# mit-han-lab/llm-awq

Measured on AMD Instinct MI355X. Metric: W4A16 decode+prefill tok/s, Llama-3-8B; achieved %HBM (GEMV) / %MFMA (GEMM), higher is better.
Workload: dtype bf16; 1 GPU; Llama-3-8B W4A16 g128 bf16 activations on 1xMI355X (decode GEMV + prefill GEMM); layers=32, decode_m=1, prefill_m=2048, graph=True, layout=cdna4, clock_ramp_steps=60, decode_mlp=gate/up + SiLU*mul launch, then down_proj, prefill_mlp=SiLU*mul fused into the gate/up GEMM epilogue, mlp=interleaved, decode_side_buffer=sz_half, parallelism=tp1, full=False

## Files before the change

### llm_awq_amd/csrc/awq_gemv_dma.hip

```cpp
#include <string.h>

#include <type_traits>
#include <utility>

#include "../../include/awq_cdna4.h"
#include "awq_device.hpp"
#include "awq_dma.hpp"
#include "awq_kernels.hpp"

namespace awq {

#ifdef AWQ_ENABLE_PROBES
#define DMA_PROBE(p) ((p) & 0xFF)
#else
#define DMA_PROBE(p) 0
#endif
constexpr int kDmaF32Out = 0x100;
constexpr int kDmaInterleave = 0x200;
template <typename DT, int WAVES, int EPI, int NS>
__device__ __forceinline__ void gemv_dma_reduce(char* smem, char* wbase, int wave_bytes, const f32x4 (&acc)[NS], const uint16_t* __restrict__ bias,
                                                uint16_t* __restrict__ out, int M, int N, int probe_, int nb, int lane, int wv) {
  const int i = lane & 15, g = lane >> 4;
#pragma unroll
  for (int s = 0; s < NS; ++s)
// ... 366 lines not shown
  if (wide8 && !g_dma_want) want = tx > 4 ? 2 : 3;
  if (g_dma_d) d = g_dma_d < tx ? g_dma_d : tx;
  while (d > 1 && dma_smem(waves, d, ns, tx, m) * want > 156 * 1024) --d;
  if (d == 3) d = 2;
  if (d == 5 || d == 6 || (d == 7 && waves == 8)) d = 4;
  if (d == 8 && waves == 16) d = 7;
  c = {waves, tx, d, dma_smem(waves, d, ns, tx, m)};
  return c.smem <= 160 * 1024 && tx >= d;
}
}

int gemv_dma_tune_set(const char* key, int value) {
  if (!strcmp(key, "gemvd_waves")) g_dma_waves = value;
  else if (!strcmp(key, "gemvd_d")) g_dma_d = value;
  else if (!strcmp(key, "gemvd_probe")) g_dma_probe = value;
  else if (!strcmp(key, "gemvd_four")) g_dma_four = value;
  else if (!strcmp(key, "gemvd_want")) g_dma_want = value;
  else if (!strcmp(key, "gemvd_wide8")) g_dma_wide8 = value;
  else if (!strcmp(key, "gemvd_il")) g_dma_il = value;
  else if (!strcmp(key, "decode_skinny_small")) g_dma_skinny_small = value;
  else if (!strcmp(key, "decode_skinny_m1")) g_dma_skinny_m1 = value;
  else if (!strcmp(key, "decode_skinny_from")) g_dma_skinny_from = value;
  else return -1;
  return 0;
}

template <typename DT, int WAVES, int D, int DQ, int EPI>
static void launch_dma_cfg(const void* x, const void* qw, const void* szp, const void* bias, void* out, int m, int n, int k,
                           const DmaCfg& c, hipStream_t st, int f32out) {
  constexpr int NS = EPI == 1 ? 2 : 1;
  const int flags = (g_dma_probe & 0xFF) | (f32out ? kDmaF32Out : 0) | ((g_dma_il == 1 || (g_dma_il == 2 && c.d < c.tx && c.waves == 8)) ? kDmaInterleave : 0);
  constexpr int TXC = EPI == 1 ? 0 : ((WAVES == 8 && (D == 2 || D == 4)) ? 4 : ((WAVES == 16 && D == 1) ? 7 : 0));
  if constexpr (TXC != 0) {
    if (m == 1 && c.tx == TXC && k == WAVES * TXC * kGroup) {
      auto kern1 = gemv_dma_kernel_m1<DT, WAVES, D, DQ, EPI, TXC>;
      static LdsOptIn optin1;
      if (c.smem > 64 * 1024) optin1.ensure(reinterpret_cast<const void*>(kern1));
      hipLaunchKernelGGL(kern1, dim3(n / 16 / NS), dim3(64 * WAVES), c.smem, st, (const uint16_t*)x, (const u32*)qw, (const u32*)szp,
                         (const uint16_t*)bias, (uint16_t*)out, m, n, k, c.tx, flags);
      return;
    }
  }
  auto kern = gemv_dma_kernel<DT, WAVES, D, DQ, EPI>;
  static LdsOptIn optin;
  if (c.smem > 64 * 1024) optin.ensure(reinterpret_cast<const void*>(kern));
  hipLaunchKernelGGL(kern, dim3(n / 16 / NS), dim3(64 * WAVES), c.smem, st, (const uint16_t*)x, (const u32*)qw, (const u32*)szp,
                     (const uint16_t*)bias, (uint16_t*)out, m, n, k, c.tx, flags);
}

template <typename DT, int EPI, int DQ>
static int launch_dma_dt(const void* x, const void* qw, const void* szp, const void* bias, void* out, int m, int n, int k,
                         hipStream_t st, int f32out) {
  DmaCfg c;
  if (!pick_dma(m, n, k, EPI == 1 ? 2 : 1, c)) return -1;
#define AWQ_DCASE(W_, D_)                                                           \
  if (c.waves == W_ && c.d == D_) {                                                 \
    launch_dma_cfg<DT, W_, D_, DQ, EPI>(x, qw, szp, bias, out, m, n, k, c, st, f32out); \
    return 0;                                                                       \
  }
  AWQ_DCASE(8, 1) AWQ_DCASE(8, 2) AWQ_DCASE(8, 4) AWQ_DCASE(8, 8)
  AWQ_DCASE(16, 1) AWQ_DCASE(16, 2) AWQ_DCASE(16, 4) AWQ_DCASE(16, 7)
  AWQ_DCASE(4, 1) AWQ_DCASE(4, 2) AWQ_DCASE(4, 4) AWQ_DCASE(4, 7) AWQ_DCASE(4, 8)
#undef AWQ_DCASE
  return -1;
}

int gemv_dma_plan(int m, int n, int k, int epi, int* kernel) {
  if (m < 1 || m > 8 || k < 128 || (k % 128) != 0 || epi < 0 || epi > 2 || n < (epi == 1 ? 32 : 16) || (n % (epi == 1 ? 32 : 16)) != 0) return 0;
  if (skinny_takes(m, n, k, epi)) {
    if (kernel) *kernel = 1;
    return 1;
  }
  if (kernel) *kernel = 0;
  DmaCfg c;
  int mc = m;
  while (mc > 1 && !pick_dma(mc, n, k, epi == 1 ? 2 : 1, c)) --mc;
  if (!pick_dma(mc, n, k, epi == 1 ? 2 : 1, c)) return 0;
  return (m + mc - 1) / mc;
}

int launch_gemv_dma(const void* x, const void* qw, const void* szp, const void* bias, void* out, int m, int n, int k, int epi,
                    int dtype, int szfmt, hipStream_t st, int f32out) {
  if (m < 1 || m > 8 || (k % 128) != 0 || (n % (epi == 1 ? 32 : 16)) != 0 || (f32out && (epi != 0 || bias != nullptr))) return -1;
  if (skinny_takes(m, n, k, epi) && launch_skinny_decode(x, qw, szp, bias, out, m, n, k, epi, dtype, szfmt, st, f32out) == 0) return 0;
  DmaCfg probe_cfg;
  int mc = m;
  while (mc > 1 && !pick_dma(mc, n, k, epi == 1 ? 2 : 1, probe_cfg)) --mc;
  if (mc < m) {
    if (!pick_dma(mc, n, k, epi == 1 ? 2 : 1, probe_cfg)) return -1;
    const size_t ncols = epi ? (size_t)n / 2 : (size_t)n;
    for (int r = 0; r < m; r += mc) {
      const int rows = m - r < mc ? m - r : mc;
      const int rc = launch_gemv_dma((const char*)x + (size_t)r * k * 2, qw, szp, bias, (char*)out + (size_t)r * ncols * (f32out ? 4 : 2), rows, n, k,
                                     epi, dtype, szfmt, st, f32out);
      if (rc != 0) return rc;
    }
    return 0;
  }
#define AWQ_DDT(DT_, DQ_)                                                                   \
  if (epi == 0) return launch_dma_dt<DT_, 0, DQ_>(x, qw, szp, bias, out, m, n, k, st, f32out); \
  if (epi == 1) return launch_dma_dt<DT_, 1, DQ_>(x, qw, szp, bias, out, m, n, k, st, 0);      \
  return launch_dma_dt<DT_, 2, DQ_>(x, qw, szp, bias, out, m, n, k, st, 0);
  if (szfmt == 1) {
    if (dtype == 0) {
      AWQ_DDT(F16, 1)
    }
    AWQ_DDT(BF16, 1)
  }
  if (dtype == 0) {
    AWQ_DDT(F16, 0)
  }
  AWQ_DDT(BF16, 0)
#undef AWQ_DDT
}

}
```

### llm_awq_amd/csrc/awq_kernels.hpp

```cpp
#pragma once
#include <hip/hip_runtime.h>
#include <stddef.h>
#include <stdint.h>

#include <atomic>

namespace awq {
struct LdsOptIn {
  std::atomic<uint64_t> done[4] = {};
  void ensure(const void* kern, int bytes = 160 * 1024) {
    int dev = 0;
    (void)hipGetDevice(&dev);
    const uint64_t bit = 1ull << (dev & 63);
    std::atomic<uint64_t>& w = done[(dev >> 6) & 3];
    if (w.load(std::memory_order_acquire) & bit) return;
    (void)hipFuncSetAttribute(kern, hipFuncAttributeMaxDynamicSharedMemorySize, bytes);
    w.fetch_or(bit, std::memory_order_release);
  }
};
inline int device_cu_count() {
  static std::atomic<int> cached[64] = {};
  int dev = 0;
  if (hipGetDevice(&dev) != hipSuccess) return 256;
  std::atomic<int>& c = cached[dev & 63];
  int v = c.load(std::memory_order_relaxed);
  if (v == 0) {
    if (hipDeviceGetAttribute(&v, hipDeviceAttributeMultiprocessorCount, dev) != hipSuccess || v <= 0) v = 256;
    c.store(v, std::memory_order_relaxed);
  }
  return v;
}
int launch_gemv(const void* x, const void* qw, const void* s, const void* z, const void* szp, void* out, int m, int n,
                int k, int dtype, int layout, hipStream_t st);
int launch_gemv_cdna4(const void* x, const void* qw, const void* szp, const void* bias, void* out, int m, int n, int k,
                      int epi, int bits, int dtype, hipStream_t st);
int launch_gemv_cdna4_norm(const void* x, const void* gamma, float eps, const void* qw, const void* szp, const void* bias, void* out,
                           int m, int n, int k, int epi, int dtype, hipStream_t st);
bool gemv_v2fast_enabled();
int launch_gemv_v2fast(const void* x, const void* qw, const void* s, const void* z, const void* bias, void* out, int m, int n, int k,
                       int gpad, int dtype, hipStream_t st);
int launch_skinny_v2(const void* x, const void* qw, const void* s, const void* z, const void* bias, void* out, int m, int n, int k,
                     int gpad, int dtype, hipStream_t st);
int launch_pack_w3(const void* q_u8, void* qw3, int n, int k, hipStream_t st);
int launch_unpack_w3(const void* qw3, void* out_u8, int n, int k, hipStream_t st);
int launch_dequant_w3(const void* qw3, const void* s, const void* z, void* out, int n, int k, int dtype, hipStream_t st);
int launch_expand_w3_to_cdna4(const void* qw3, void* qw4, int n, int k, hipStream_t st);
int gemv_cdna4_tune_set(const char* key, int value);
int launch_gemv_dma(const void* x, const void* qw, const void* szp, const void* bias, void* out, int m, int n, int k, int epi,
                    int dtype, int szfmt, hipStream_t st, int f32out = 0);
int gemv_dma_tune_set(const char* key, int value);
int launch_moe_gemv_cdna4(const void* x, const void* qw, const void* szp, const void* offsets, void* out, int total_rows,
                          int experts, int n, int k, int dtype, hipStream_t st);
int launch_moe_skinny_tail_cdna4(const void* x, const void* qw, const void* szp, const void* offsets, void* out, int experts, int n, int k,
                                 int dtype, hipStream_t st, int epi, int tail);
void moe_v6_set_tail(int v);
int launch_moe_skinny_cdna4(const void* x, const void* qw, const void* szp, const void* offsets, void* out, int total_rows,
                            int experts, int n, int k, int dtype, hipStream_t st);
int launch_pack_sz_cdna4(const void* s, const void* z, void* szp, int n, int k, hipStream_t st);
int launch_pack_szh_cdna4(const void* s, const void* z, void* szh, int* inexact, int n, int k, int dtype, hipStream_t st);
int launch_gemm(const void* x, const void* qw, const void* s, const void* z, const void* szp, void* out, int m, int n,
                int k, int dtype, int layout, void* ws, size_t ws_bytes, hipStream_t st);
int launch_repack_v2_cdna4(const void* src, void* dst, int n, int k, int to_cdna4, hipStream_t st);
int launch_unpack_cdna4(const void* qw, void* out_u8, int n, int k, hipStream_t st);
int launch_dequant_cdna4(const void* qw, const void* s, const void* z, void* out, int n, int k, int dtype, hipStream_t st);
size_t gemm_workspace_bytes(int m, int n, int k);
int launch_gemm_cdna4_v3(const void* x, const void* qw, const void* szp, const void* bias, void* out, int m, int n, int k,
                         int tile_n, int dtype, void* ws, size_t ws_bytes, hipStream_t st, int bits = 4, int epi = 0, const void* szh = nullptr);
int gemm_variant_get();
int launch_skinny_cdna4(const void* x, const void* qw, const void* szp, const void* bias, void* out, int m, int n, int k,
                        int dtype, hipStream_t st, int f32out = 0, void* ws = nullptr, size_t ws_bytes = 0);
int launch_skinny_w3(const void* x, const void* qw, const void* szp, const void* bias, void* out, int m, int n, int k, int epi, int dtype, hipStream_t st,
                     int f32out = 0);
int launch_skinny_gate_up(const void* x, const void* qw, const void* szp, void* out, int m, int n2, int k, int dtype, hipStream_t st);
int skinny_splitk_parts(int m, int n, int k);
size_t skinny_splitk_workspace_bytes(int m, int n, int k);
int skinny_tune_set(const char* key, int value);
int launch_midm_cdna4(const void* x, const void* qw, const void* szp, const void* bias, void* out, int m, int n, int k, int epi, int dtype, int szfmt,
                      int bits, int f32out, void* ws, size_t ws_bytes, hipStream_t st);
bool midm_takes(int m, int n, int k);
size_t midm_workspace_bytes(int m, int n, int k);
int midm_parts(int m, int n, int k);
int midm_tune_set(const char* key, int value);
int midm_init();
unsigned* splitk_ticket_words(hipStream_t st, int groups);
int launch_skinny_decode(const void* x, const void* qw, const void* szp, const void* bias, void* out, int m, int n, int k, int epi,
                         int dtype, int szfmt, hipStream_t st, int f32out = 0);
int launch_moe_gemm(const void* x, const void* qw, const void* s, const void* z, const void* offsets, void* out, int total_m,
                    int experts, int n, int k, int gpad, int dtype, int layout, hipStream_t st);
int gemv_tune_set(const char* key, int value);
int gemm_tune_set(const char* key, int value);
int gemm_v3_tune_set(const char* key, int value);
void launch_gemm_cdna4_v4n(const void* x, const void* qw, const void* szp, const void* bias, void* out, int m, int n, int k,
                           int n_begin, int n_end, int dtype, void* ws, size_t ws_bytes, hipStream_t st, int bits = 4, int epi = 0);
size_t gemm_v4n_workspace_bytes(int m, int n_cols, int k);
extern int g_v4n_ksplit_force;
extern int g_v4n_ksplit_cap;
bool gemm_cdna4_v3_takes(int m, int k);
size_t gemm_cdna4_v3_workspace_bytes(int m, int n, int k);
int gemm_cdna4_v3_plan(int m, int n, int bits, int* mode, int* cols_main);
int gemm_cdna4_v3_narrow_kernel(int m, int n_cols, int k, int bits, int has_workspace, int epi);
int gemv_dma_plan(int m, int n, int k, int epi, int* kernel);
size_t gemm_cdna4_v3_workspace_bytes_w3(int m, int n, int k);
bool moe_v4_enabled();
int launch_moe_gemm_cdna4_v6(const void* x, const void* qw, const void* szp, const void* offsets, void* out, int total, int experts,
                             int n, int k, int dtype, hipStream_t st, int epi = 0, const void* szh = nullptr);
int launch_silu_mul_interleaved(const void* in, void* out, int m, int n2, int dtype, hipStream_t st);
int launch_silu_mul(const void* gate, const void* up, void* out, size_t count, int dtype, hipStream_t st);
bool moe_v6_enabled();
int launch_moe_route(const void* logits, int logits_dtype, int tokens, int experts, int top_k, int renormalize, void* topk_ids, void* topk_w,
                     void* order, void* inv, void* offsets, hipStream_t st);
int launch_moe_gather(const void* x, const void* order, void* xs, int tokens, int top_k, int hidden, hipStream_t st);
int launch_moe_combine(const void* ys, const void* inv, const void* topk_w, void* out, int tokens, int top_k, int hidden, int dtype, hipStream_t st);
int launch_sample_logits(const void* logits, int logits_dtype, int batch, int vocab, const void* u, const void* temperature, const void* top_k,
                         const void* top_p, const void* penalty, void* history, void* hist_len, int max_history, void* seqlens, const void* stop_ids,
                         int num_stop, void* finished, int max_len, int flags, void* tokens, hipStream_t st);
int launch_spec_draft_ngram(const void* history, const void* hist_len, const void* seqlens, const void* max_draft, void* drafts, void* draft_len,
                            int batch, int max_history, int vocab, int kmax, int ngram_min, int ngram_max, int max_len, hipStream_t st);
int launch_spec_pack(const void* last_tokens, void* drafts, void* draft_len, const void* seqlens, void* cu_seqlens_q, void* input_ids, int batch,
                     int kmax, int total_q, hipStream_t st);
int launch_spec_verify(const void* logits, int logits_dtype, int total_q, int vocab, const void* u, const void* cu_seqlens_q, const void* input_ids,
                       int batch, const void* temperature, const void* top_k, const void* top_p, const void* penalty, const void* history,
                       const void* hist_len, int max_history, void* row_tokens, hipStream_t st);
int launch_spec_accept(const void* row_tokens, const void* input_ids, const void* cu_seqlens_q, int batch, int total_q, int kmax, void* history,
                       void* hist_len, int max_history, void* seqlens, const void* stop_ids, int num_stop, void* finished, int max_len, int flags,
                       void* out_tokens, void* num_emitted, void* last_tokens, hipStream_t st);
int lm_head_plan(int m, int v, int k, int out[4]);
int launch_lm_head(const void* x, long ldx, const void* gamma, float eps, const void* weight, const void* bias, const int* seqlens, void* out,
                   int out_f32, int m, int v, int k, int dtype, int max_blocks, hipStream_t st);
int launch_embed_tokens(const int* tokens, const void* table, void* out, int n, int v, int k, hipStream_t st);
int lora_plan(int k, int r, int n_slices, int out[4]);
size_t lora_workspace_bytes(int total_q, int k, int r, int n_slices);
int launch_lora_shrink(const void* x, long ldx, const void* a_pool, const int* adapter_ids, const int* cu_seqlens_q, void* ws, int batch,
                       int max_seqlen_q, int total_q, int slots, int k, int r, int n_slices, int dtype, hipStream_t st);
int launch_lora_expand(const void* ws, const void* b_pool, const float* scaling, const int* adapter_ids, const int* cu_seqlens_q, void* y, int batch,
                       int max_seqlen_q, int total_q, int slots, int n, int k, int r, const int* slice_end, int n_slices, int dtype, hipStream_t st);
int launch_lora_expand_gate_up(const void* ws, const void* b_pool, const float* scaling, const int* adapter_ids, const int* cu_seqlens_q,
                               const void* y2, void* h, int batch, int max_seqlen_q, int total_q, int slots, int n2, int k, int r, int dtype,
                               hipStream_t st);
int launch_quantize_group(const void* w, long ldw, const void* col_scale, const void* clip_max, void* w_fake, void* scales, void* scaled_zeros,
                          void* zeros, void* qweight, int layout, int n, int k, int n_bit, int dtype, hipStream_t st);
void quantize_group_host(const void* w, long ldw, const void* col_scale, const void* clip_max, void* w_fake, void* scales, void* scaled_zeros,
                         void* zeros, void* intweight, int n, int k, int n_bit, int dtype);
int launch_clip_search(const void* w, long ldw, const void* x, long ldx, void* best_max_val, int* best_idx, float* err, int n, int k, int s,
                       int n_bit, int n_grid, int n_steps, int dtype, hipStream_t st);
void launch_gemm_cdna4_v6(const void* x, const void* qw, const void* szp, const void* bias, void* out, int m, int n, int k, int n_begin,
                          int n_end, int dtype, hipStream_t st, int bits = 4, int epi = 0, int szfmt = 0, int tile_n = 256);
void gemm_v6_set_probe(int v);
bool gemm_v6_pair_takes(int m, int n, int k);
int gemm_v6_pair_lost(unsigned* count);
int gemm_cdna4_v3_pair_plan(int m, int n, int k);
size_t gemm_v6_pair_workspace_bytes(int m, int n, int k);
int launch_gemm_cdna4_v6_pair(const void* x, const void* qw, const void* szp, const void* bias, void* out, int m, int n, int k, int n_begin, int n_end,
                              int dtype, void* ws, size_t ws_bytes, hipStream_t st, int bits = 4, int epi = 0, int szfmt = 0);
void gemm_v6_set_pair_lead(int v);
void gemm_v6_set_pair_min_nit(int v);
int launch_bias_add(void* out, const void* bias, int m, int n, int dtype, hipStream_t st);
int launch_round_bias_f32(const void* in_f32, const void* bias, void* out, int m, int n, int dtype, hipStream_t st);
int launch_rmsnorm(const void* x, const void* gamma, float eps, void* out, int m, int k, int dtype, hipStream_t st);
int attn_decode_plan(int batch, int nheads_kv, int head_dim, int timestep, int lmax, int* splits, int* chunk);
size_t attn_decode_workspace_bytes(int batch, int nheads, int nheads_kv, int head_dim, int timestep, int lmax);
int launch_attn_decode(const void* q, const void* k, const void* v, void* k_cache, void* v_cache, const int* lens, const float* alibi,
                       void* out, int B, int H, int Hkv, int Dh, int Lmax, long long q_bs, long long k_bs, long long v_bs, int timestep,
                       int rot, float rot_base, float rot_scale, int neox, int dtype, void* workspace, hipStream_t st);
int attn_prefill_plan(int batch, int nheads, int nheads_kv, int head_dim, int seqlen_q, int seqlen_k, int causal, int* q_tile_rows,
                      int* blocks);
int attn_varq_plan(int batch, int nheads, int nheads_kv, int head_dim, int max_seqlen_q, int* q_tile_rows, int* blocks);
int attn_prefill_tune_set(const char* key, int value);
int launch_attn_prefill(const void* q, const void* k, const void* v, void* out, int B, int Sq, int Sk, int H, int Hkv, int Dh, long long q_bs,
                        long long q_rs, long long k_bs, long long k_rs, long long v_bs, long long v_rs, float scale, int causal, int dtype,
// ... 38 lines not shown
```

### llm_awq_amd/csrc/awq_skinny_cdna4.hip

```cpp
#include <string.h>

#include <atomic>

#include "awq_device.hpp"
#include "awq_kernels.hpp"

namespace awq {

template <typename DT, int WAVES, int NS, int CB, int DQ = 0, int EPI = 0, int BITS = 4, int XU = 4 * CB>
__device__ __forceinline__ void skinny_cdna4_body(char* smem, const uint16_t* __restrict__ x, const u32* __restrict__ qw,
                                                  const u32* __restrict__ szp, const uint16_t* __restrict__ bias,
                                                  uint16_t* __restrict__ out, int M, int N, int K, int nb, int f32out = 0, int k0 = 0, int kn = -1) {
  using vec8 = typename DT::vec8;
  constexpr int XB = 4 * CB;
  constexpr int XBYTES = 16 * CB * 256;
  const int lane = threadIdx.x & 63, wv = __builtin_amdgcn_readfirstlane(threadIdx.x >> 6);
  const int i = lane & 15, g = lane >> 4;
  const int nit = K >> 7, nslab = N >> 4;
  char* xs = smem + wv * XBYTES;

  static_assert(BITS == 4 || DQ == 0, "the w3c tiles have no sz_half form");
  constexpr u32 kTile = BITS == 4 ? 1024u : 768u;
  const __amdgpu_buffer_rsrc_t rw = __builtin_amdgcn_make_buffer_rsrc(const_cast<u32*>(qw), 0, nslab * nit * (int)kTile, 0x00020000);
  const __amdgpu_buffer_rsrc_t rs = __builtin_amdgcn_make_buffer_rsrc(const_cast<u32*>(szp), 0, nslab * nit * 64, 0x00020000);
  const __amdgpu_buffer_rsrc_t rx = __builtin_amdgcn_make_buffer_rsrc(const_cast<uint16_t*>(x), 0, M * K * 2, 0x00020000);
  u32 slab_tile[NS];
#pragma unroll
  for (int s = 0; s < NS; ++s) slab_tile[s] = (u32)min(nb * NS + s, nslab - 1) * (u32)nit;
  const u32 wlane_b = BITS == 4 ? lane * 16u : lane * 12u, ilane_b = (u32)i * 4u;
  u32 xsrc_b[XB];
#pragma unroll
  for (int b = 0; b < XB; ++b) {
    const int r = 4 * b + g;
    xsrc_b[b] = ((u32)min(r, M - 1) * (u32)K + (u32)((i ^ (r & 15)) * 8)) * 2u;
  }

  Cdna4DequantT<DT> cd;
  Cdna4DequantH<DT> ch;
  if (DQ == 0) cd.init(lane, BITS == 4 ? 0x000F000Fu : 0x00070007u);
  else ch.init(lane);
  if (kn < 0) kn = nit;
  const int cnt = (kn - wv + WAVES - 1) / WAVES;

  f32x4 acc[NS][CB];
#pragma unroll
  for (int s = 0; s < NS; ++s)
#pragma unroll
    for (int c = 0; c < CB; ++c) acc[s][c] = f32x4{0.f, 0.f, 0.f, 0.f};

  u32x4 w[NS], xr[XB];
  u32 sz[NS];
  auto load_step = [&](int t) {
    const int kg = k0 + min(wv + WAVES * t, kn - 1);
#pragma unroll
    for (int b = 0; b < XU; ++b) xr[b] = __builtin_amdgcn_raw_buffer_load_b128(rx, xsrc_b[b], (u32)kg * 256u, 0);
#pragma unroll
    for (int s = 0; s < NS; ++s) {
      const u32 tidx = slab_tile[s] + (u32)kg;
      if (BITS == 4) {
        w[s] = __builtin_amdgcn_raw_buffer_load_b128(rw, wlane_b, tidx * 1024u, 2);
      } else {
        typedef u32 u32x3 __attribute__((ext_vector_type(3)));
        const u32x3 w3 = __builtin_amdgcn_raw_buffer_load_b96(rw, wlane_b, tidx * 768u, 2);
        w[s] = u32x4{w3.x, w3.y, w3.z, 0u};
      }
      sz[s] = __builtin_amdgcn_raw_buffer_load_b32(rs, ilane_b, tidx * 64u, 0);
    }
  };
  if (cnt > 0) load_step(0);
  for (int t = 0; t < cnt; ++t) {
#pragma unroll
    for (int b = 0; b < XU; ++b) *reinterpret_cast<u32x4*>(xs + b * 1024 + lane * 16) = xr[b];
    u32x4 wc[NS];
    u32 szc[NS];
#pragma unroll
    for (int s = 0; s < NS; ++s) {
      wc[s] = w[s];
      szc[s] = sz[s];
    }
    if (t + 1 < cnt) load_step(t + 1);
    vec8 xo[CB][4];
#pragma unroll
    for (int c = 0; c < CB; ++c) {
      const char* xrow = xs + (c * 16 + i) * 256;
#pragma unroll
      for (int a = 0; a < 4; ++a) xo[c][a] = *reinterpret_cast<const vec8*>(xrow + (((4 * a + g) ^ i) << 4));
    }
#pragma unroll
    for (int s = 0; s < NS; ++s) {
      vec8 op[4];
      if (DQ == 0) cd.tile_packed(BITS == 4 ? wc[s] : w3_expand(wc[s].x, wc[s].y, wc[s].z), szc[s], op);
      else ch.tile(wc[s], szc[s], op);
#pragma unroll
      for (int a = 0; a < 4; ++a)
#pragma unroll
        for (int c = 0; c < CB; ++c) acc[s][c] = DT::mfma(op[a], xo[c][a], acc[s][c]);
    }
  }

  __syncthreads();
  float* red = reinterpret_cast<float*>(smem);
  constexpr int NBLK = NS * CB;
#pragma unroll
  for (int s = 0; s < NS; ++s)
#pragma unroll
    for (int c = 0; c < CB; ++c)
#pragma unroll
      for (int r = 0; r < 4; ++r) red[((wv * NBLK + s * CB + c) * 4 + r) * 64 + lane] = acc[s][c][r];
  __syncthreads();
  for (int blk = wv; blk < NBLK; blk += WAVES) {
    const int s = blk / CB, c = blk - s * CB;
    const int slab = nb * NS + s, m = 16 * c + i;
    float v[4];
#pragma unroll
    for (int r = 0; r < 4; ++r) {
      float t = 0.f;
#pragma unroll
      for (int q = 0; q < WAVES; ++q) t += red[((q * NBLK + blk) * 4 + r) * 64 + lane];
      v[r] = t;
    }
    auto to_f = [](uint16_t b) { return DT::to_float(b); };
    if (EPI == 2) {
      float u[4];
#pragma unroll
      for (int r = 0; r < 4; ++r) {
        float t = 0.f;
#pragma unroll
        for (int q = 0; q < WAVES; ++q) t += red[((q * NBLK + blk) * 4 + r) * 64 + ((lane + 32) & 63)];
        u[r] = t;
      }
      if (slab < nslab && m < M && g < 2) {
        uint16_t o[4];
#pragma unroll
        for (int r = 0; r < 4; ++r) {
          const float gt = to_f(DT::from_float(v[r])), up = to_f(DT::from_float(u[r]));
          const float sl = to_f(DT::from_float(silu_f32(gt)));
          o[r] = DT::from_float(sl * up);
        }
        *reinterpret_cast<u32x2*>(out + (size_t)m * (N >> 1) + slab * 8 + 4 * g) =
            u32x2{(u32)o[0] | ((u32)o[1] << 16), (u32)o[2] | ((u32)o[3] << 16)};
      }
    } else if (f32out) {
      if (slab < nslab && m < M) {
        float* dst = reinterpret_cast<float*>(out) + (size_t)m * N + slab * 16 + 4 * g;
        const f32x4 pv = f32x4{v[0], v[1], v[2], v[3]};
        if (f32out == 2) asm volatile("global_store_dwordx4 %0, %1, off sc1\n\ts_nop 1" : : "v"(dst), "v"(pv) : "memory");
        else *reinterpret_cast<f32x4*>(dst) = pv;
      }
    } else if (slab < nslab && m < M) {
      const int nn = slab * 16 + 4 * g;
      uint16_t o[4];
#pragma unroll
      for (int r = 0; r < 4; ++r) {
        o[r] = DT::from_float(v[r]);
        if (bias != nullptr) o[r] = DT::from_float(to_f(o[r]) + to_f(bias[nn + r]));
      }
      *reinterpret_cast<u32x2*>(out + (size_t)m * N + nn) = u32x2{(u32)o[0] | ((u32)o[1] << 16), (u32)o[2] | ((u32)o[3] << 16)};
    }
  }
}

template <typename DT, int WAVES, int NS, int CB, int DQ = 0, int EPI = 0, int BITS = 4, int XU = 4 * CB>
__global__ __launch_bounds__(64 * WAVES) void skinny_cdna4_kernel(const uint16_t* __restrict__ x, const u32* __restrict__ qw,
                                                                   const u32* __restrict__ szp,
                                                                   const uint16_t* __restrict__ bias,
                                                                   uint16_t* __restrict__ out, int M, int N, int K, int f32out) {
  extern __shared__ __attribute__((aligned(16))) char smem[];
  skinny_cdna4_body<DT, WAVES, NS, CB, DQ, EPI, BITS, XU>(smem, x, qw, szp, bias, out, M, N, K, blockIdx.x, EPI == 0 ? f32out : 0);
}

constexpr int kMoeTailMaxExperts = 64;
template <typename DT, int WAVES, int NS, int CB, int EPI = 0>
__global__ __launch_bounds__(64 * WAVES) void moe_skinny_cdna4_kernel(const uint16_t* __restrict__ x, const u32* __restrict__ qw,
                                                                       const u32* __restrict__ szp,
                                                                       const int* __restrict__ offsets,
                                                                       uint16_t* __restrict__ out, int N, int K, int groups, int experts, int tail_lo, int tail) {
  extern __shared__ __attribute__((aligned(16))) char smem[];
  const size_t et = (size_t)(N >> 4) * (K >> 7);
  const int ncol = EPI == 2 ? (N >> 1) : N;
  if (tail > 0) {
    auto qualifies = [&](int e2) {
      const int rem = (offsets[e2 + 1] - offsets[e2]) & 255;
      return rem >= tail_lo && rem < tail;
    };
    int nq = 0;
    for (int e2 = 0; e2 < experts; ++e2) nq += qualifies(e2) ? 1 : 0;
    for (int item = blockIdx.x; item < nq * groups; item += gridDim.x) {
      const int q = item / groups, nb = item - q * groups;
      int e = 0;
      for (int seen = 0; e < experts; ++e) {
        if (qualifies(e)) {
          if (seen == q) break;
          ++seen;
        }
      }
      const int lo = offsets[e], cnt = offsets[e + 1] - lo, rem = cnt & 255;
      skinny_cdna4_body<DT, WAVES, NS, CB, 0, EPI>(smem, x + (size_t)(lo + cnt - rem) * K, qw + (size_t)e * et * 256, szp + (size_t)e * et * 16, nullptr,
                                                   out + (size_t)(lo + cnt - rem) * ncol, rem, N, K, nb);
      __syncthreads();
    }
    return;
  }
  const int e = blockIdx.x / groups, nb = blockIdx.x - e * groups;
  const int row0 = offsets[e], m_e = offsets[e + 1] - row0;
  for (int r0 = 0; r0 < m_e; r0 += 16 * CB) {
    if (r0 > 0) __syncthreads();
    skinny_cdna4_body<DT, WAVES, NS, CB, 0, EPI>(smem, x + (size_t)(row0 + r0) * K, qw + (size_t)e * et * 256, szp + (size_t)e * et * 16, nullptr,
                                                 out + (size_t)(row0 + r0) * ncol, min(m_e - r0, 16 * CB), N, K, nb);
  }
}

template <typename DT, int WAVES, int NS, int CB, int DQ = 0, int EPI = 0, int BITS = 4, int XU = 4 * CB>
static void launch_skinny(const void* x, const void* qw, const void* szp, const void* bias, void* out, int m, int n, int k,
                          hipStream_t st, int f32out = 0) {
  const size_t xbytes = (size_t)WAVES * 16 * CB * 256, rbytes = (size_t)WAVES * NS * CB * 1024;
  const size_t smem = xbytes > rbytes ? xbytes : rbytes;
  auto kern = skinny_cdna4_kernel<DT, WAVES, NS, CB, DQ, EPI, BITS, XU>;
  static LdsOptIn optin;
  if (smem > 64 * 1024) optin.ensure(reinterpret_cast<const void*>(kern));
  const int nslab = n / 16;
  hipLaunchKernelGGL(kern, dim3((nslab + NS - 1) / NS), dim3(64 * WAVES), smem, st, (const uint16_t*)x, (const u32*)qw,
                     (const u32*)szp, (const uint16_t*)bias, (uint16_t*)out, m, n, k, f32out);
}

template <typename DT, int WAVES, int NS, int CB, int DQ = 0>
__global__ __launch_bounds__(64 * WAVES) void skinny_splitk_kernel(const uint16_t* __restrict__ x, const u32* __restrict__ qw,
                                                                   const u32* __restrict__ szp, const uint16_t* __restrict__ bias,
                                                                   uint16_t* __restrict__ out, float* __restrict__ parts, u32* __restrict__ tickets,
                                                                   int M, int N, int K) {
  extern __shared__ __attribute__((aligned(16))) char smem[];
  const int nb = blockIdx.x, KS = gridDim.y, p = blockIdx.y, kn = (K >> 7) / KS;
  skinny_cdna4_body<DT, WAVES, NS, CB, DQ, 0>(smem, x, qw, szp, nullptr, reinterpret_cast<uint16_t*>(parts + (size_t)p * M * N), M, N, K, nb, 2, p * kn, kn);
  asm volatile("s_waitcnt vmcnt(0)" : : : "memory");
  __syncthreads();
  u32* bc = reinterpret_cast<u32*>(smem);
  if (threadIdx.x == 0) bc[0] = __hip_atomic_fetch_add(tickets + nb, 1u, __ATOMIC_RELAXED, __HIP_MEMORY_SCOPE_AGENT);
  __syncthreads();
  if (bc[0] != (u32)(KS - 1)) return;
  if (threadIdx.x == 0) __hip_atomic_store(tickets + nb, 0u, __ATOMIC_RELAXED, __HIP_MEMORY_SCOPE_AGENT);
  constexpr int QC = NS * 4;
  const int nslab = N >> 4;
  for (int idx = threadIdx.x; idx < M * QC; idx += 64 * WAVES) {
    const int m = idx / QC, q = idx - m * QC, col = nb * NS * 16 + 4 * q;
    if (col >= nslab * 16) continue;
    f32x4 acc = f32x4{0.f, 0.f, 0.f, 0.f};
    for (int p0 = 0; p0 < KS; p0 += 4) {
      f32x4 v[4];
#pragma unroll
      for (int j = 0; j < 4; ++j) {
        const float* src = parts + ((size_t)min(p0 + j, KS - 1) * M + m) * N + col;
        asm volatile("global_load_dwordx4 %0, %1, off sc1" : "=v"(v[j]) : "v"(src) : "memory");
// ... 122 lines not shown
  if (!szp || m < 9 || m > 64 || (n2 % 32) != 0 || (k % 128) != 0 || (size_t)m * (size_t)k >= (1ull << 31)) return -1;
  if (dtype == 0) return launch_skinny_64<F16, 2>(x, qw, szp, nullptr, out, m, n2, k, st, 0, nullptr, 0);
  return launch_skinny_64<BF16, 2>(x, qw, szp, nullptr, out, m, n2, k, st, 0, nullptr, 0);
}

template <typename DT, int EPI>
static void launch_skinny_w3_dt(const void* x, const void* qw, const void* szp, const void* bias, void* out, int m, int n, int k, hipStream_t st, int f32out) {
  const int nslab = n / 16;
  const bool wide = nslab >= 512;
  if (m <= 16) {
    if (wide) launch_skinny<DT, 8, 2, 1, 0, EPI, 3>(x, qw, szp, bias, out, m, n, k, st, f32out);
    else launch_skinny<DT, 8, 1, 1, 0, EPI, 3>(x, qw, szp, bias, out, m, n, k, st, f32out);
  } else if (m <= 32) {
    if (wide) launch_skinny<DT, 8, 2, 2, 0, EPI, 3>(x, qw, szp, bias, out, m, n, k, st, f32out);
    else launch_skinny<DT, 8, 1, 2, 0, EPI, 3>(x, qw, szp, bias, out, m, n, k, st, f32out);
  } else {
    if (wide) launch_skinny<DT, 4, 4, 4, 0, EPI, 3>(x, qw, szp, bias, out, m, n, k, st, f32out);
    else launch_skinny<DT, 8, 2, 4, 0, EPI, 3>(x, qw, szp, bias, out, m, n, k, st, f32out);
  }
}
int launch_skinny_w3(const void* x, const void* qw, const void* szp, const void* bias, void* out, int m, int n, int k, int epi, int dtype, hipStream_t st,
                     int f32out) {
  if (!szp || m < 9 || m > 64 || (n % (epi == 2 ? 32 : 16)) != 0 || (k % 128) != 0 || (epi != 0 && epi != 2) || (epi == 2 && bias) ||
      (f32out && (epi != 0 || bias)) || (size_t)m * (size_t)k >= (1ull << 31))
    return -1;
  if (dtype == 0) {
    if (epi == 2) launch_skinny_w3_dt<F16, 2>(x, qw, szp, nullptr, out, m, n, k, st, 0);
    else launch_skinny_w3_dt<F16, 0>(x, qw, szp, bias, out, m, n, k, st, f32out);
  } else {
    if (epi == 2) launch_skinny_w3_dt<BF16, 2>(x, qw, szp, nullptr, out, m, n, k, st, 0);
    else launch_skinny_w3_dt<BF16, 0>(x, qw, szp, bias, out, m, n, k, st, f32out);
  }
  return 0;
}

int launch_skinny_decode(const void* x, const void* qw, const void* szp, const void* bias, void* out, int m, int n, int k, int epi,
                         int dtype, int szfmt, hipStream_t st, int f32out) {
  if (!szp || m < 1 || m > 16 || (n % 16) != 0 || (k % 128) != 0 || (epi != 0 && epi != 2) || (epi == 2 && bias) || (f32out && (epi || bias))) return -1;
  const bool wide = n / 16 >= 1024, deep = !wide && (k / 128 >= 96 || (g_skinny_deep64 && m <= 8 && k / 128 >= g_skinny_deep64 && n / 16 <= device_cu_count()));
#define AWQ_SD(DT_, DQ_, EPI_)                                                                    \
  {                                                                                               \
    if (m <= 4 && g_skinny_xu) {   \
      if (wide && seven_slab_round(n / 16)) launch_skinny<DT_, 8, 7, 1, DQ_, EPI_, 4, 1>(x, qw, szp, bias, out, m, n, k, st, f32out); \
      else if (wide) launch_skinny<DT_, 8, 2, 1, DQ_, EPI_, 4, 1>(x, qw, szp, bias, out, m, n, k, st, f32out);       \
      else if (deep) launch_skinny<DT_, 16, 1, 1, DQ_, EPI_, 4, 1>(x, qw, szp, bias, out, m, n, k, st, f32out); \
      else launch_skinny<DT_, 8, 1, 1, DQ_, EPI_, 4, 1>(x, qw, szp, bias, out, m, n, k, st, f32out);            \
      return 0;                                                                                   \
    }                                                                                             \
    if (m <= 8 && g_skinny_xu) {   \
      if (wide && seven_slab_round(n / 16)) launch_skinny<DT_, 8, 7, 1, DQ_, EPI_, 4, 2>(x, qw, szp, bias, out, m, n, k, st, f32out); \
      else if (wide) launch_skinny<DT_, 8, 2, 1, DQ_, EPI_, 4, 2>(x, qw, szp, bias, out, m, n, k, st, f32out);       \
      else if (deep) launch_skinny<DT_, 16, 1, 1, DQ_, EPI_, 4, 2>(x, qw, szp, bias, out, m, n, k, st, f32out); \
      else launch_skinny<DT_, 8, 1, 1, DQ_, EPI_, 4, 2>(x, qw, szp, bias, out, m, n, k, st, f32out);            \
      return 0;                                                                                   \
    }                                                                                             \
    if (m <= 12 && g_skinny_xu) {   \
      if (wide && seven_slab_round(n / 16)) launch_skinny<DT_, 8, 7, 1, DQ_, EPI_, 4, 3>(x, qw, szp, bias, out, m, n, k, st, f32out); \
      else if (wide) launch_skinny<DT_, 8, 2, 1, DQ_, EPI_, 4, 3>(x, qw, szp, bias, out, m, n, k, st, f32out);       \
      else if (deep) launch_skinny<DT_, 16, 1, 1, DQ_, EPI_, 4, 3>(x, qw, szp, bias, out, m, n, k, st, f32out); \
      else launch_skinny<DT_, 8, 1, 1, DQ_, EPI_, 4, 3>(x, qw, szp, bias, out, m, n, k, st, f32out);            \
      return 0;                                                                                   \
    }                                                                                             \
    if (wide && seven_slab_round(n / 16)) launch_skinny<DT_, 8, 7, 1, DQ_, EPI_>(x, qw, szp, bias, out, m, n, k, st, f32out); \
    else if (wide) launch_skinny<DT_, 8, 2, 1, DQ_, EPI_>(x, qw, szp, bias, out, m, n, k, st, f32out);       \
    else if (deep) launch_skinny<DT_, 16, 1, 1, DQ_, EPI_>(x, qw, szp, bias, out, m, n, k, st, f32out); \
    else launch_skinny<DT_, 8, 1, 1, DQ_, EPI_>(x, qw, szp, bias, out, m, n, k, st, f32out);            \
    return 0;                                                                                     \
  }
#define AWQ_SD_DT(DT_)                          \
  if (szfmt == 1) {                             \
    if (epi == 2) AWQ_SD(DT_, 1, 2)             \
    AWQ_SD(DT_, 1, 0)                           \
  }                                             \
  if (epi == 2) AWQ_SD(DT_, 0, 2)               \
  AWQ_SD(DT_, 0, 0)
  if (dtype == 0) {
    AWQ_SD_DT(F16)
  }
  AWQ_SD_DT(BF16)
#undef AWQ_SD_DT
#undef AWQ_SD
}

template <typename DT, int WAVES, int NS, int CB, int EPI = 0>
static void launch_moe_skinny(const void* x, const void* qw, const void* szp, const void* offsets, void* out, int experts, int n, int k,
                              hipStream_t st, int tail_lo = 0, int tail = 0) {
  const size_t xbytes = (size_t)WAVES * 16 * CB * 256, rbytes = (size_t)WAVES * NS * CB * 1024;
  const size_t smem = xbytes > rbytes ? xbytes : rbytes;
  auto kern = moe_skinny_cdna4_kernel<DT, WAVES, NS, CB, EPI>;
  static LdsOptIn optin;
  if (smem > 64 * 1024) optin.ensure(reinterpret_cast<const void*>(kern));
  const int groups = (n / 16 + NS - 1) / NS;
  int blocks = experts * groups;
  if (tail > 0) {
    const int per_cu = smem <= 32 * 1024 ? 4 : (smem <= 64 * 1024 ? 2 : 1);
    const int cap = device_cu_count() * per_cu;
    if (blocks > cap) blocks = cap;
  }
  hipLaunchKernelGGL(kern, dim3(blocks), dim3(64 * WAVES), smem, st, (const uint16_t*)x, (const u32*)qw, (const u32*)szp,
                     (const int*)offsets, (uint16_t*)out, n, k, groups, experts, tail_lo, tail);
}

int launch_moe_skinny_tail_cdna4(const void* x, const void* qw, const void* szp, const void* offsets, void* out, int experts, int n, int k,
                                 int dtype, hipStream_t st, int epi, int tail) {
  if (!szp || experts < 1 || experts > kMoeTailMaxExperts || (n % 16) != 0 || (k % 128) != 0 || tail < 1 || tail > 64 || (epi != 0 && epi != 2) ||
      (epi == 2 && (n % 32) != 0))
    return -1;
  if ((size_t)n * (size_t)k / 8 >= (1ull << 31)) return -1;
#define AWQ_MST(DT_, EPI_)                                                                                              \
  {                                                                                                                     \
    launch_moe_skinny<DT_, 8, 2, 1, EPI_>(x, qw, szp, offsets, out, experts, n, k, st, 1, tail < 17 ? tail : 17);       \
    if (tail > 17) launch_moe_skinny<DT_, 8, 2, 2, EPI_>(x, qw, szp, offsets, out, experts, n, k, st, 17, tail < 33 ? tail : 33); \
    if (tail > 33) launch_moe_skinny<DT_, 8, 2, 4, EPI_>(x, qw, szp, offsets, out, experts, n, k, st, 33, tail);        \
  }
  if (dtype == 0) {
    if (epi == 2) AWQ_MST(F16, 2) else AWQ_MST(F16, 0)
  } else {
    if (epi == 2) AWQ_MST(BF16, 2) else AWQ_MST(BF16, 0)
  }
#undef AWQ_MST
  return 0;
}

int launch_moe_skinny_cdna4(const void* x, const void* qw, const void* szp, const void* offsets, void* out, int total_rows,
                            int experts, int n, int k, int dtype, hipStream_t st) {
  if (!szp || total_rows < 1 || total_rows > 255 || experts < 1 || (n % 16) != 0 || (k % 128) != 0) return -1;
  if ((size_t)n * (size_t)k / 8 >= (1ull << 31) || (size_t)total_rows * (size_t)k >= (1ull << 31)) return -1;
  const int want = (3 * total_rows + 2 * experts - 1) / (2 * experts);
  const int cb = want <= 16 ? 1 : (want <= 32 ? 2 : (want <= 48 ? 3 : 4));
  const bool wide = n / 16 >= 512;
#define AWQ_MS(DT_)                                                                                             \
  if (cb == 1) {                                                                                                \
    if (wide) launch_moe_skinny<DT_, 8, 2, 1>(x, qw, szp, offsets, out, experts, n, k, st);                     \
    else launch_moe_skinny<DT_, 8, 1, 1>(x, qw, szp, offsets, out, experts, n, k, st);                          \
  } else if (cb == 2) {                                                                                         \
    if (wide) launch_moe_skinny<DT_, 8, 2, 2>(x, qw, szp, offsets, out, experts, n, k, st);                     \
    else launch_moe_skinny<DT_, 8, 1, 2>(x, qw, szp, offsets, out, experts, n, k, st);                          \
  } else if (cb == 3) {                                                                                         \
    launch_moe_skinny<DT_, 8, 2, 3>(x, qw, szp, offsets, out, experts, n, k, st);                               \
  } else {                                                                                                      \
    launch_moe_skinny<DT_, 8, 2, 4>(x, qw, szp, offsets, out, experts, n, k, st);                               \
  }
  if (dtype == 0) {
    AWQ_MS(F16)
  } else {
    AWQ_MS(BF16)
  }
#undef AWQ_MS
  return 0;
}

}
```

Measured before the change: 1027 decode tok/s (the 160 quantised linears of one token: 32 x {qkv, o, gate, up, down}; attention/norm/lm_head off-path).

## Add specialised single-row decode GEMV kernel with hand-scheduled buffer loads

Adds a dedicated M=1 kernel for epi-0 linears whose K is 4096 or 8192. Each wave issues all its weight and scale buffer loads up front with non-temporal hints and DMAs x into LDS. It then double-buffers the x LDS reads and scale prep across K steps, using explicit vmcnt waits before a cross-wave LDS reduction. The dispatcher tries it ahead of the generic skinny decode path only when a flag bit is set. The aim is lower per-GEMV latency and better HBM streaming for the qkv and o projections, at the cost of inline-asm fragility and extra kernel variants.

```diff
diff --git a/llm_awq_amd/csrc/awq_gemv_dma.hip b/llm_awq_amd/csrc/awq_gemv_dma.hip
--- a/llm_awq_amd/csrc/awq_gemv_dma.hip
+++ b/llm_awq_amd/csrc/awq_gemv_dma.hip
@@ -472,7 +472,10 @@
 int launch_gemv_dma(const void* x, const void* qw, const void* szp, const void* bias, void* out, int m, int n, int k, int epi,
                     int dtype, int szfmt, hipStream_t st, int f32out) {
   if (m < 1 || m > 8 || (k % 128) != 0 || (n % (epi == 1 ? 32 : 16)) != 0 || (f32out && (epi != 0 || bias != nullptr))) return -1;
-  if (skinny_takes(m, n, k, epi) && launch_skinny_decode(x, qw, szp, bias, out, m, n, k, epi, dtype, szfmt, st, f32out) == 0) return 0;
+  if (skinny_takes(m, n, k, epi)) {
+    if (m == 1 && epi == 0 && !f32out && (g_dma_skinny_m1 & 4) && launch_skinny_one_row(x, qw, szp, bias, out, n, k, dtype, szfmt, st) == 0) return 0;
+    if (launch_skinny_decode(x, qw, szp, bias, out, m, n, k, epi, dtype, szfmt, st, f32out) == 0) return 0;
+  }
   DmaCfg probe_cfg;
   int mc = m;
   while (mc > 1 && !pick_dma(mc, n, k, epi == 1 ? 2 : 1, probe_cfg)) --mc;
diff --git a/llm_awq_amd/csrc/awq_kernels.hpp b/llm_awq_amd/csrc/awq_kernels.hpp
--- a/llm_awq_amd/csrc/awq_kernels.hpp
+++ b/llm_awq_amd/csrc/awq_kernels.hpp
@@ -85,6 +85,7 @@
 unsigned* splitk_ticket_words(hipStream_t st, int groups);
 int launch_skinny_decode(const void* x, const void* qw, const void* szp, const void* bias, void* out, int m, int n, int k, int epi,
                          int dtype, int szfmt, hipStream_t st, int f32out = 0);
+int launch_skinny_one_row(const void* x, const void* qw, const void* szp, const void* bias, void* out, int n, int k, int dtype, int szfmt, hipStream_t st);
 int launch_moe_gemm(const void* x, const void* qw, const void* s, const void* z, const void* offsets, void* out, int total_m,
                     int experts, int n, int k, int gpad, int dtype, int layout, hipStream_t st);
 int gemv_tune_set(const char* key, int value);
diff --git a/llm_awq_amd/csrc/awq_skinny_cdna4.hip b/llm_awq_amd/csrc/awq_skinny_cdna4.hip
--- a/llm_awq_amd/csrc/awq_skinny_cdna4.hip
+++ b/llm_awq_amd/csrc/awq_skinny_cdna4.hip
@@ -1,8 +1,10 @@
 #include <string.h>
 
 #include <atomic>
+#include <type_traits>
 
 #include "awq_device.hpp"
+#include "awq_dma.hpp"
 #include "awq_kernels.hpp"
 
 namespace awq {
@@ -167,6 +169,138 @@
                                                                    uint16_t* __restrict__ out, int M, int N, int K, int f32out) {
   extern __shared__ __attribute__((aligned(16))) char smem[];
   skinny_cdna4_body<DT, WAVES, NS, CB, DQ, EPI, BITS, XU>(smem, x, qw, szp, bias, out, M, N, K, blockIdx.x, EPI == 0 ? f32out : 0);
+}
+
+__device__ __forceinline__ u32x4 one_row_rsrc(const void* p, u32 bytes) {
+  const unsigned long long a = reinterpret_cast<unsigned long long>(p);
+  return u32x4{(u32)a, (u32)(a >> 32) & 0xFFFFu, bytes, 0x00020000u};
+}
+template <int XO>
+__device__ __forceinline__ void one_row_read_x(u32x4 (&xo)[4], u32 x_lane) {
+  asm volatile("ds_read_b128 %0, %4 offset:%5\n\tds_read_b128 %1, %4 offset:%6\n\tds_read_b128 %2, %4 offset:%7\n\tds_read_b128 %3, %4 offset:%8"
+               : "=&v"(xo[0]), "=&v"(xo[1]), "=&v"(xo[2]), "=&v"(xo[3])
+               : "v"(x_lane), "n"(XO), "n"(XO + 64), "n"(XO + 128), "n"(XO + 192)
+               : "memory");
+}
+__device__ __forceinline__ void one_row_load_w(u32x4& w, u32 voff, const u32x4& rsrc, u32 soff) {
+  asm volatile("buffer_load_dwordx4 %0, %1, %2, %3 offen nt" : "=v"(w) : "v"(voff), "s"(rsrc), "s"(soff) : "memory");
+}
+template <int OFF>
+__device__ __forceinline__ void one_row_load_sz(u32& sz, u32 voff, const u32x4& rsrc, u32 soff) {
+  asm volatile("buffer_load_dword %0, %1, %2, %3 offen offset:%4" : "=v"(sz) : "v"(voff), "s"(rsrc), "s"(soff), "n"(OFF) : "memory");
+}
+template <int VM>
+__device__ __forceinline__ void one_row_wait_w(u32x4& w) {
+  asm volatile("s_waitcnt vmcnt(%1)" : "+v"(w) : "n"(VM) : "memory");
+}
+template <int TX>
+__device__ __forceinline__ void one_row_wait_head(u32x4& w0, u32 (&sz)[TX]) {
+  if constexpr (TX == 4)
+    asm volatile("s_waitcnt vmcnt(3)" : "+v"(w0), "+v"(sz[0]), "+v"(sz[1]), "+v"(sz[2]), "+v"(sz[3]) : : "memory");
+  else
+    asm volatile("s_waitcnt vmcnt(7)"
+                 : "+v"(w0), "+v"(sz[0]), "+v"(sz[1]), "+v"(sz[2]), "+v"(sz[3]), "+v"(sz[4]), "+v"(sz[5]), "+v"(sz[6]), "+v"(sz[7])
+                 :
+                 : "memory");
+}
+template <typename DT>
+__device__ __forceinline__ void one_row_wait_x(u32x4 (&xo)[4], typename Cdna4DequantT<DT>::Prep& p) {
+  asm volatile("s_waitcnt lgkmcnt(0)" : "+v"(xo[0]), "+v"(xo[1]), "+v"(xo[2]), "+v"(xo[3]), "+v"(p.cv) : : "memory");
+}
+template <typename DT>
+__device__ __forceinline__ void one_row_wait_x(u32x4 (&xo)[4], typename Cdna4DequantH<DT>::Prep& p) {
+  asm volatile("s_waitcnt lgkmcnt(0)" : "+v"(xo[0]), "+v"(xo[1]), "+v"(xo[2]), "+v"(xo[3]), "+v"(p.c), "+v"(p.b) : : "memory");
+}
+template <typename DT, int WAVES, int TX, int DQ>
+__device__ __forceinline__ void skinny_one_row_body(char* smem, const uint16_t* __restrict__ x, const u32* __restrict__ qw, const u32* __restrict__ szp,
+                                                    const uint16_t* __restrict__ bias, uint16_t* __restrict__ out, int N, int nb) {
+  using vec8 = typename DT::vec8;
+  constexpr int nit = WAVES * TX, K = nit * 128, NP = TX / 4;
+  constexpr int wave_bytes = TX * 256 > 1024 ? TX * 256 : 1024;
+  static_assert(TX % 4 == 0 && TX <= 8, "x arrives in four-step pieces; the scale dwords sit at immediate offsets");
+  const int lane = threadIdx.x & 63, wv = __builtin_amdgcn_readfirstlane(threadIdx.x >> 6);
+  const int i = lane & 15, g = lane >> 4;
+  const int nslab = N >> 4;
+  char* wbase = smem + wv * wave_bytes;
+  const u32x4 rw = one_row_rsrc(qw, (u32)nslab * (u32)nit * 1024u), rs = one_row_rsrc(szp, (u32)nslab * (u32)nit * 64u);
+  const __amdgpu_buffer_rsrc_t rx = __builtin_amdgcn_make_buffer_rsrc(const_cast<uint16_t*>(x), 0, K * 2, 0x00020000);
+  const u32 tile0 = (u32)nb * (u32)nit + (u32)wv;
+  const u32 wlane_b = lane * 16u, ilane_b = (u32)i * 4u, x_voff = (u32)g * (u32)(WAVES * 256) + (u32)i * 16u;
+
+  u32x4 w[TX];
+  u32 sz[TX];
+  one_row_load_w(w[0], wlane_b, rw, tile0 * 1024u);
+#pragma unroll
+  for (int q = 0; q < NP; ++q) dma_to_lds<16, 0>(rx, wbase + q * 1024, x_voff, (u32)(wv + WAVES * 4 * q) * 256u);
+  static_for<0, TX>([&](auto t_) {
+    constexpr int T = decltype(t_)::value;
+    one_row_load_sz<WAVES * T * 64>(sz[T], ilane_b, rs, tile0 * 64u);
+  });
+  static_for<1, TX>([&](auto t_) {
+    constexpr int T = decltype(t_)::value;
+    one_row_load_w(w[T], wlane_b, rw, (tile0 + (u32)(WAVES * T)) * 1024u);
+  });
+
+  Cdna4DequantT<DT> cd;
+  Cdna4DequantH<DT> ch;
+  if (DQ == 0) cd.init(lane);
+  else ch.init(lane);
+  using Prep = std::conditional_t<DQ == 0, typename Cdna4DequantT<DT>::Prep, typename Cdna4DequantH<DT>::Prep>;
+  auto prep = [&](u32 s) {
+    if constexpr (DQ == 0) return cd.prep(s);
+    else return ch.prep_lean(s);
+  };
+  const u32 x_lane = (u32)(size_t)(__attribute__((address_space(3))) char*)wbase + (u32)g * 16u;
+
+  f32x4 acc = f32x4{0.f, 0.f, 0.f, 0.f};
+  u32x4 xo[2][4];
+  Prep pp[2];
+  one_row_wait_head<TX>(w[0], sz);
+  one_row_read_x<0>(xo[0], x_lane);
+  pp[0] = prep(sz[0]);
+  static_for<0, TX>([&](auto t_) {
+    constexpr int T = decltype(t_)::value, H = T & 1;
+    one_row_wait_x<DT>(xo[H], pp[H]);
+    if constexpr (T + 1 < TX) {
+      one_row_read_x<(T + 1) * 256>(xo[H ^ 1], x_lane);
+      pp[H ^ 1] = prep(sz[T + 1]);
+    }
+    const u32 ws[4] = {w[T].x, w[T].y, w[T].z, w[T].w};
+    vec8 op[4];
+#pragma unroll
+    for (int a = 0; a < 4; ++a) {
+      if constexpr (DQ == 0) op[a] = cd.word(ws[a], pp[H]);
+      else op[a] = ch.word(ws[a], pp[H]);
+    }
+#pragma unroll
+    for (int a = 0; a < 4; ++a) acc = DT::mfma(op[a], __builtin_bit_cast(vec8, xo[H][a]), acc);
+    if constexpr (T + 1 < TX) {
+      __builtin_amdgcn_sched_barrier(0);
+      one_row_wait_w<TX - 2 - T>(w[T + 1]);
+    }
+  });
+  __builtin_amdgcn_sched_barrier(0);
+
+#pragma unroll
+  for (int r = 0; r < 4; ++r) reinterpret_cast<float*>(wbase)[r * 64 + lane] = acc[r];
+  __syncthreads();
+  if (wv < 4 && i == 0) {
+    const int r = wv;
+    float v = 0.f;
+#pragma unroll
+    for (int q = 0; q < WAVES; ++q) v += reinterpret_cast<const float*>(smem + q * wave_bytes)[r * 64 + lane];
+    const int nn = nb * 16 + 4 * g + r;
+    uint16_t o = DT::from_float(v);
+    if (bias != nullptr) o = DT::from_float(DT::to_float(o) + DT::to_float(bias[nn]));
+    out[nn] = o;
+  }
+}
+
+template <typename DT, int WAVES, int TX, int DQ>
+__global__ __launch_bounds__(64 * WAVES) void skinny_one_row_kernel(const uint16_t* __restrict__ x, const u32* __restrict__ qw, const u32* __restrict__ szp,
+                                                                     const uint16_t* __restrict__ bias, uint16_t* __restrict__ out, int N) {
+  extern __shared__ __attribute__((aligned(16))) char smem[];
+  skinny_one_row_body<DT, WAVES, TX, DQ>(smem, x, qw, szp, bias, out, N, blockIdx.x);
 }
 
 constexpr int kMoeTailMaxExperts = 64;
@@ -455,6 +589,31 @@
 #undef AWQ_SD
 }
 
+template <typename DT, int TX, int DQ>
+static void launch_one_row(const void* x, const void* qw, const void* szp, const void* bias, void* out, int n, hipStream_t st) {
+  constexpr size_t smem = 8 * (size_t)(TX * 256 > 1024 ? TX * 256 : 1024);
+  hipLaunchKernelGGL((skinny_one_row_kernel<DT, 8, TX, DQ>), dim3(n / 16), dim3(64 * 8), smem, st, (const uint16_t*)x, (const u32*)qw, (const u32*)szp,
+                     (const uint16_t*)bias, (uint16_t*)out, n);
+}
+int launch_skinny_one_row(const void* x, const void* qw, const void* szp, const void* bias, void* out, int n, int k, int dtype, int szfmt, hipStream_t st) {
+  const int nslab = n / 16, tx = k / (8 * 128);
+  if (!szp || (n % 16) != 0 || k != tx * 8 * 128 || (tx != 4 && tx != 8)) return -1;
+  if (nslab >= 1024 || (g_skinny_deep64 && k / 128 >= g_skinny_deep64 && nslab <= device_cu_count())) return -1;
+#define AWQ_OR(DT_, DQ_)                                                  \
+  {                                                                       \
+    if (tx == 4) launch_one_row<DT_, 4, DQ_>(x, qw, szp, bias, out, n, st); \
+    else launch_one_row<DT_, 8, DQ_>(x, qw, szp, bias, out, n, st);       \
+    return 0;                                                             \
+  }
+  if (dtype == 0) {
+    if (szfmt == 1) AWQ_OR(F16, 1)
+    AWQ_OR(F16, 0)
+  }
+  if (szfmt == 1) AWQ_OR(BF16, 1)
+  AWQ_OR(BF16, 0)
+#undef AWQ_OR
+}
+
 template <typename DT, int WAVES, int NS, int CB, int EPI = 0>
 static void launch_moe_skinny(const void* x, const void* qw, const void* szp, const void* offsets, void* out, int experts, int n, int k,
                               hipStream_t st, int tail_lo = 0, int tail = 0) {
```

New measurement: 1015 decode tok/s (the 160 quantised linears of one token: 32 x {qkv, o, gate, up, down}; attention/norm/lm_head off-path). -1.2%, worse.
